# itailang/geometric_adv

Measured on AMD Instinct MI355X. Metric: attack-iterations/sec (B=32, N=2048) at 1/2/4/8 GPUs; Chamfer rel-err vs ref, higher is better.
Workload: dtype f32 (encoder products: f16x2); 1 GPU; BASELINE configs[1]: B=32 random clouds x N=2048, output-space attack (chamfer/chamfer, dist_weight 1.0, lr 0.01), one batch per GPU; batch_per_gpu=32, n_points=2048, global_batch=32, parallelism=batches sharded, dp1, no data-path collective, ranks=1, collective_backend=none, collective_world=1

## Files before the change

geometric_adv_amd/adv_ae.py:

```python
import ctypes as C
import time

import numpy as np
import torch

from . import _lib
from .adversary import init_pert_value
from .autoencoder import PointNetAE


class Configuration:

    def __init__(self, batch_size, n_points, weights, loss="chamfer", loss_adv_type="chamfer",
                 loss_dist_type="chamfer", dist_weight_list=(1.0,), max_point_pert_weight=0.0,
                 max_point_dist_weight=0.0, num_iterations=500, num_iterations_thresh=400,
                 learning_rate=0.01, ae_name="autoencoder", emd_weight=0.0, verbose=False, batch_slots=1,
                 chamfer_prune=True, emd_reference_weights=False, recompute_backward=False, separate_adam=False,
                 chamfer_kernel="auto", encoder_backward="auto", emd_dense_levels=False, encoder_arith=None, loss_in_scan=True):
        self.batch_size = int(batch_size)
        self.n_input = [int(n_points), 3]
        self.n_output = [int(n_points), 3]
        self.weights = weights
        self.loss = loss
        self.loss_adv_type = loss_adv_type
# ... 142 lines not shown
            return None
        if 2 * handed_back > self.B:
            self.set_source_search(False)
        return handed_back

    def status(self):
        with torch.cuda.device(self.device):
            _lib.check(_lib.lib().geoadv_attack_status(self._h, _lib.stream_handle()), "attack_status")

    def peek(self):
        B, n, dev = self.B, self.n, self.device
        f = lambda *s: torch.empty(s, dtype=torch.float32, device=dev)
        i = lambda *s: torch.empty(s, dtype=torch.int32, device=dev)
        out = dict(pert=f(B, n, 3), adv=f(B, n, 3), recon=f(B, n, 3), latent=f(B, 128), grad=f(B, n, 3),
                   idx_r1=i(B, n), idx_r2=i(B, n), idx_a1=i(B, n), idx_a2=i(B, n))
        with torch.cuda.device(dev):
            _lib.check(_lib.lib().geoadv_attack_peek(self._h, *[_lib.ptr(out[k]) for k in
                       ("pert", "adv", "recon", "latent", "grad", "idx_r1", "idx_r2", "idx_a1", "idx_a2")],
                       _lib.stream_handle()), "attack_peek")
        if self.ae.bneck != 128:
            out["latent"] = out["latent"][:, :self.ae.bneck].contiguous()
        return out

    def profile(self, classes, stride=1):
        _lib.check(_lib.lib().geoadv_attack_profile_stride(self._h, int(stride)), "attack_profile_stride")
        if classes is True:
            mask = -1
        elif not classes:
            mask = 0
        else:
            mask = sum(1 << PROF_NAMES.index(c) for c in classes)
        _lib.check(_lib.lib().geoadv_attack_profile(self._h, int(mask)), "attack_profile")

    def markers(self, enable=True):
        _lib.check(_lib.lib().geoadv_attack_markers(self._h, int(bool(enable))), "attack_markers")

    def profile_read(self):
        out = {}
        for k, name in enumerate(PROF_NAMES):
            n_, ms = C.c_int(0), C.c_float(0)
            _lib.check(_lib.lib().geoadv_attack_profile_read(self._h, k, C.byref(n_), C.byref(ms)), "attack_profile_read")
            out[name] = (n_.value, ms.value)
        return out

    def reconstruct(self, X, GT=None, compute_loss=True):
        return self.ae.reconstruct(X, GT, compute_loss)
# ... 100 lines not shown
```

geometric_adv_amd/csrc/attack.hip:

```cpp
#include "ae.h"
#include "chamfer_sym.h"
#include "chamfer_grad.h"
#include "chamfer_grid.h"
#include "encoder_jac.h"
#include "decoder_tail.h"
#define LC_STAMP(K, I) GA_STAMP(K, I)
#include "loss_cgrad.h"
#include <dlfcn.h>
#include <limits.h>
#include <math.h>
#include <stdlib.h>
#include <vector>

#pragma clang fp contract(off)

namespace geoadv {

struct ChamferScan { const float *query; const float *target; float *dist; int *idx; int nq, nt; const int *need; };
int launch_chamfer_scans(const ChamferScan *scans, int nscan, int b, hipStream_t stream);
int launch_encoder_jac(const DeviceAE &A, int b, const JacArgs &a, hipStream_t stream);
int launch_encoder_bwd_dense(const DeviceAE &A, int b, const float *adv, const float *z, const int *zcnt, const float *dz,
                             const int *dense_flag, float *g_enc, hipStream_t stream);
int launch_decoder_fc2_bwd(const DeviceAE &A, int b, const float *g_recon, float *partial, hipStream_t stream);
int launch_decoder_tail_dense(const DeviceAE &A, const TailDenseArgs &a, hipStream_t stream);
// ... 40 lines not shown
    r = block_reduce(r, shf, shi);
    if (t == 0) out[b] = r.s3 * (1.0f / (float)n) + r.s4 * (1.0f / (float)m);
}

__global__ __launch_bounds__(CGA_THREADS) void chamfer_grad_attack_kernel(CGradArgs a) {
    extern __shared__ __attribute__((aligned(16))) unsigned lds[];
    const CGradProblem pr = a.pr[blockIdx.y];
    const int b = blockIdx.x, n = a.n;
    const float wb = pr.w ? pr.w[b] : 1.0f;
    const float gd = wb * (1.0f / (float)n);
    GradSide s;
    s.n_own = n; s.n_oth = n;
    s.own = pr.p + (size_t)b * n * 3; s.oth = pr.q + (size_t)b * n * 3;
    s.match_own = pr.idx1 + (size_t)b * n; s.match_oth = pr.idx2 + (size_t)b * n;
    s.gd_own = nullptr; s.gd_oth = nullptr; s.gd_own_s = gd; s.gd_oth_s = gd;
    s.jstar = (pr.jstar && pr.extra_w > 0.f) ? pr.jstar[b] : -1;
    s.extra = wb * pr.extra_w;
    s.gout = pr.g + (size_t)b * n * 3;
    chamfer_grad_side<true, CGA_THREADS>(s, lds, a.P);
}

__global__ __launch_bounds__(CGA_THREADS) void chamfer_grad_attack_fx_kernel(CGradArgs a, int H) {
    extern __shared__ __attribute__((aligned(16))) unsigned fx_lds[];
    cgrad_fx_body(a, blockIdx.y / H, blockIdx.x, blockIdx.y % H, H, fx_lds);
}

__global__ __launch_bounds__(CGA_THREADS) void loss_cgrad_kernel(LossArgs la, CGradArgs ca, int H) {
    extern __shared__ __attribute__((aligned(16))) unsigned lc_lds[];
    GA_STAMP(0, 0);
    loss_cgrad_block(la, ca, H, blockIdx.x, gridDim.x, blockIdx.y, lc_lds);
    GA_STAMP(0, 7);
}

struct AdamArgs {
    int n, B;
    float *pert, *m, *v;
    float *g_enc;
    const float *g_dist;
    const float *w, *losses;
    const int *jstar;
    int loss_dist_type;
    float mp_pert_w;
    float alpha, one_minus_b1, one_minus_b2, eps;
    float *grad_out;
    const float *x;
    float *adv_out;
};
// ... 59 lines not shown
    }
}

}

using namespace geoadv;

struct geoadv_attack {
    const geoadv_ae *ae;
    geoadv_attack_config cfg;
    int B, n;
    void *arena; size_t arena_bytes;
    float *x, *gt, *tz, *w;
    float *pert, *m, *v;
    float *adv, *recon, *g_recon, *g_dist, *g_enc, *grad_last;
    float *r1, *r2, *a1, *a2; int *ir1, *ir2, *ia1, *ia2;
    ForwardScratch fs;
    float *dz, *dec_partial;
    float *losses; int *jstar;
    float *best_err, *best_metrics, *best_adv, *best_recon;
    float *emd_temp, *emd_cost, *emd_g1;
    float *sym_ws;
    unsigned long long *row64;
    bool row64_filled;
    bool cgrad_done;
    bool counted = false;
    bool chamfer_prune;
    int *need_adv[2];
    float *x_box;
    int grid_calls;
    unsigned *masks;
    float *jac;
    bool jac_valid;
    unsigned *tail_ready;
    unsigned tail_epoch;
    unsigned *loss_done;
    unsigned loss_target;
    bool host_loss_force;
    bool host_loss;
    int cus;
    bool chamfer_sym;
    float beta1_pow, beta2_pow;
    bool fwd_valid;
    bool adv_valid;
    bool fuse_adam;
    bool adam_pending;
// ... 61 lines not shown
    ~ProfScope() {
        if (marked) roctx().pop();
        if (!on) return;
        if (!kernel) {
            e1 = at->ev_used++;
            (void)hipEventRecord(at->ev[e1], st);
        }
        at->marks.push_back({which, e0, e1});
    }
};


int do_forward(geoadv_attack *at, float *hist_slot, int keep, hipStream_t st) {
    const DeviceAE &A = at->ae->d;
    const int B = at->B, n = at->n;
    const ChamferScan sc_recon[2] = {{at->recon, at->gt, at->r1, at->ir1, n, n}, {at->gt, at->recon, at->r2, at->ir2, n, n}};
    const ChamferScan sc_adv[2] = {{at->adv, at->x, at->a1, at->ia1, n, n}, {at->x, at->adv, at->a2, at->ia2, n, n}};
    const bool pruned = at->chamfer_prune && chamfer_grid_supports(n, n);
    const bool adv_chamfer = at->cfg.loss_adv_type == GEOADV_LOSS_ADV_CHAMFER;
    const bool dist_chamfer = at->cfg.loss_dist_type == GEOADV_LOSS_DIST_CHAMFER;
    const bool max_term = dist_chamfer && at->cfg.max_point_dist_weight > 0.f;
    const bool loss_fused = (adv_chamfer || dist_chamfer) && !max_term && n <= CG_FX_MAX_N_PLANE;
    const bool merge_in_loss = loss_fused && adv_chamfer && dist_chamfer;
    const bool use_row64 = merge_in_loss && at->chamfer_sym && at->row64 != nullptr && chamfer_sym_packs_rows((long)B * (pruned ? 1 : 2), n, n);
    SymPartials part{nullptr, nullptr, 1, B, false, use_row64 ? at->row64 : nullptr};
    {
        ProfScope ps(at, GEOADV_PROF_ENCODER_FWD, st, true);
        if (int rc = launch_encoder_fwd(A, B, at->x, at->pert, (at->adv_valid && !at->adam_pending) ? nullptr : at->adv, at->fs.pmax,
                                        at->fs.parg, at->fs.pcnt, at->masks, st, ps.start(), ps.stop(),
                                        at->adam_pending ? &at->pending : nullptr)) return rc;
        at->adam_pending = false;
        at->adv_valid = true;
    }
    const bool rides_scan = pruned && chamfer_grid_rides(n) && at->chamfer_sym;
    const bool rides_latent = pruned && chamfer_grid_rides(n) && !at->chamfer_sym;
    const int call = at->grid_calls;
    int *need_new = at->need_adv[rides_scan ? (call + 1) & 1 : 0];
    const int *need_scan = at->need_adv[rides_scan ? call & 1 : 0];
    if (pruned) at->grid_calls++;
    {
        ProfScope ps(at, GEOADV_PROF_DECODER_FWD, st);
        if (pruned && !rides_scan && !rides_latent) {
            if (int rc = launch_chamfer_grid(at->adv, at->x, at->a1, at->ia1, at->a2, at->ia2, B, n, need_new, call, at->x_box, st)) return rc;
        }
        if (rides_latent) {
            if (int rc = launch_latent_decode_and_grid(A, B, at->fs.pmax, at->fs.parg, at->fs.pcnt, at->fs.z, at->fs.crit, at->fs.zcnt,
                                                       at->fs.dense, at->fs.d1, at->fs.d2, at->adv, at->x, at->a1, at->ia1, at->a2,
                                                       at->ia2, n, need_new, call, at->x_box, st)) return rc;
        } else if (int rc = launch_latent_decode(A, B, at->fs.pmax, at->fs.parg, at->fs.pcnt, at->fs.z, at->fs.crit, at->fs.zcnt,
                                                 at->fs.dense, at->fs.d1, at->fs.d2, st)) return rc;
        if (int rc = launch_decoder_fc2(A, B, at->fs.d2, at->recon, st, use_row64 ? at->row64 : nullptr, use_row64 ? 2 * (size_t)B * n : 0)) return rc;
    }
    const JacArgs jargs{n, at->masks, at->fs.crit, at->fs.z, at->fs.dense, at->jac};
    const bool jac_rides = at->jac && at->chamfer_sym;
    at->jac_valid = jac_rides;
    if (at->jac && !jac_rides && at->cfg.encoder_backward == GEOADV_ENC_BWD_JACOBIAN) {
        ProfScope ps(at, GEOADV_PROF_ENCODER_BWD, st);
        if (int rc = launch_encoder_jac(A, B, jargs, st)) return rc;
        at->jac_valid = true;
    }
    auto fill_loss = [&](const SymPartials &p, LossArgs &la, CGradArgs &ca, int &np) {
        la.n = n; la.loss_adv_type = at->cfg.loss_adv_type; la.loss_dist_type = at->cfg.loss_dist_type;
        la.mp_pert_w = at->cfg.max_point_pert_weight; la.mp_dist_w = at->cfg.max_point_dist_weight;
        la.r1 = at->r1; la.r2 = at->r2; la.a1 = at->a1; la.a2 = at->a2; la.pert = at->pert;
        la.z = at->fs.z; la.tz = at->tz; la.w = at->w; la.losses = at->losses; la.jstar = at->jstar;
        la.emd_cost = at->emd_temp ? at->emd_cost : nullptr; la.emd_weight = at->cfg.emd_weight;
        la.dz_latent = at->dz; la.hist = hist_slot; la.keep = keep; la.best_err = at->best_err;
        la.best_metrics = at->best_metrics; la.adv = at->adv; la.recon = at->recon;
        la.best_adv = at->best_adv; la.best_recon = at->best_recon;
        la.part = p; la.a1_need = pruned ? need_scan : nullptr; la.a1_all = pruned ? 0 : 1; la.r1_out = at->r1; la.a1_out = at->a1;
        np = 0;
        if (adv_chamfer) {
            ca.pr[np] = CGradProblem{at->recon, at->gt, at->ir1, at->ir2, at->g_recon, nullptr, nullptr, 0.f};
            if (p.deferred) {
                ca.pr[np].part_d = p.rowpart_d; ca.pr[np].part_i = p.rowpart_i; ca.pr[np].part_slices = p.slices;
                ca.pr[np].part_need = nullptr; ca.pr[np].idx1_out = at->ir1; ca.pr[np].part_w = p.row64;
            }
            ++np;
        }
        if (dist_chamfer) {
            ca.pr[np] = CGradProblem{at->adv, at->x, at->ia1, at->ia2, at->g_dist, at->w, at->jstar, 0.f};
            if (p.deferred) {
                const size_t off = (size_t)B * p.slices * n;
                ca.pr[np].part_d = p.rowpart_d + off; ca.pr[np].part_i = p.rowpart_i + off; ca.pr[np].part_slices = p.slices;
                ca.pr[np].part_need = pruned ? need_scan : nullptr; ca.pr[np].idx1_out = at->ia1;
                ca.pr[np].part_w = p.row64 ? p.row64 + (size_t)B * n : nullptr;
            }
            ++np;
        }
        ca.n = n; ca.P = 0;
    };
    struct LossCtx { void (*fill)(void *, const SymPartials &, LossArgs &, CGradArgs &, int &); void *self; };
// ... 364 lines not shown

extern "C" int geoadv_attack_get_best(geoadv_attack *at, const float *target_ae_loss_ref, float *metrics, float *adv,
                                      float *recon, void *stream) {
    GA_REQUIRE(at, "attack_get_best: null handle");
    hipStream_t st = as_stream(stream);
    const size_t bn3 = (size_t)at->B * at->n * 3;
    if (metrics) {
        GA_REQUIRE(target_ae_loss_ref, "attack_get_best: target_ae_loss_ref is required for the metrics");
        best_metrics_kernel<<<(at->B + 63) / 64, 64, 0, st>>>(at->B, at->best_metrics, at->best_err, target_ae_loss_ref, metrics,
                                                              reinterpret_cast<const int *>(at->tail_ready + at->B));
        GA_LAUNCH_CHECK();
    }
    if (adv) GA_HIP(hipMemcpyAsync(adv, at->best_adv, 4 * bn3, hipMemcpyDeviceToDevice, st));
    if (recon) GA_HIP(hipMemcpyAsync(recon, at->best_recon, 4 * bn3, hipMemcpyDeviceToDevice, st));
    return GEOADV_OK;
}

extern "C" int geoadv_attack_set_source_search(geoadv_attack *at, int on) {
    GA_REQUIRE(at, "attack_set_source_search: null handle");
    at->chamfer_prune = on != 0;
    return GEOADV_OK;
}

extern "C" int geoadv_attack_status(geoadv_attack *at, void *stream) {
    GA_REQUIRE(at, "attack_status: null handle");
    hipStream_t st = as_stream(stream);
    int failed = 0;
    GA_HIP(hipMemcpyAsync(&failed, at->tail_ready + at->B, sizeof(int), hipMemcpyDeviceToHost, st));
    GA_HIP(hipStreamSynchronize(st));
    if (failed) {
        set_error("attack: an in-launch hand-off (decoder backward tail -> dense encoder backward of a cloud with a tied pool "
                  "maximum) timed out since the last set_inputs / init_pert; iterations after it used a stale latent gradient -- "
                  "the results of this run are invalid");
        return GEOADV_EHIP;
    }
    return ae_range_check(at->ae, st, "attack_status");
}

extern "C" int geoadv_attack_peek(geoadv_attack *at, float *pert, float *adv, float *recon, float *latent, float *grad,
                                  int *idx_r1, int *idx_r2, int *idx_a1, int *idx_a2, void *stream) {
    GA_REQUIRE(at, "attack_peek: null handle");
    hipStream_t st = as_stream(stream);
    const size_t bn3 = 4 * (size_t)at->B * at->n * 3, bn = 4 * (size_t)at->B * at->n;
    if (at->adam_pending || (!at->fwd_valid && (adv || recon || latent || idx_r1 || idx_r2 || idx_a1 || idx_a2)))
        if (int rc = do_forward(at, nullptr, 0, st)) return rc;
    if (pert) GA_HIP(hipMemcpyAsync(pert, at->pert, bn3, hipMemcpyDeviceToDevice, st));
// ... 65 lines not shown
```

geometric_adv_amd/csrc/chamfer_sym.h:

```cpp
#pragma once
#include "common.h"

namespace geoadv {

struct ChamferPair {
    const float *p, *q;
    float *dist1; int *idx1;
    float *dist2; int *idx2;
};

struct SymPartials {
    const float *rowpart_d;
    const int *rowpart_i;
    int slices, clouds;
    bool deferred;
    unsigned long long *row64;
};

#ifdef __HIPCC__
__device__ __forceinline__ bool sym_needed(const int *need, int c) {
    if (!need) return true;
    const int4 lo = reinterpret_cast<const int4 *>(need)[2 * c], hi = reinterpret_cast<const int4 *>(need)[2 * c + 1];
    return (lo.x | lo.y | lo.z | lo.w | hi.x | hi.y | hi.z | hi.w) != 0;
}

__device__ __forceinline__ float sym_merge_pick(const float *d, int slices, size_t stride, int &slice) {
    float bd = d[0];
    int bs = 0;
    for (int s0 = 1; s0 < slices; s0 += 8) {
        float vd[8];
#pragma unroll
        for (int u = 0; u < 8; ++u) vd[u] = d[(size_t)(s0 + u < slices ? s0 + u : 0) * stride];
#pragma unroll
        for (int u = 0; u < 8; ++u)
            if (s0 + u < slices && vd[u] < bd) { bd = vd[u]; bs = s0 + u; }
    }
    slice = bs;
    return bd;
}
// ... 14 lines not shown
#pragma unroll
        for (int u = 0; u < 8; ++u) bd = fminf(bd, vd[u]);
    }
    return bd;
}
#endif

struct CGradProblem {
    const float *p, *q;
    const int *idx1, *idx2;
    float *g;
    const float *w;
    const int *jstar;
    float extra_w;
    const float *part_d; const int *part_i; int part_slices; const int *part_need; int *idx1_out;
    const unsigned long long *part_w;
};
int launch_chamfer_grad(const CGradProblem *pr, int np, int B, int n, hipStream_t st);

int launch_nn_nonfinite_fix(int b, int n, const float *xyz1, int m, const float *xyz2, float *dist1, int *idx1, float *dist2,
                            int *idx2, hipStream_t stream);

size_t chamfer_sym_workspace_floats(int pairs, int b, int n, int m);
bool chamfer_sym_packs_rows(long live_groups, int n, int m);
int launch_chamfer_sym(const ChamferPair *pairs, int np, int b, int n, int m, float *workspace, hipStream_t stream);
struct GridArgs;
struct JacRider;
struct LossRider;
int launch_chamfer_sym_loop(const ChamferPair *pairs, int np, int b, int n, int m, float *workspace, const int *need1,
                            const GridArgs *rider, const JacRider *jac, SymPartials *defer, hipStream_t stream, LossRider *loss = nullptr);
bool chamfer_sym_hosts_loss(long live_groups, int b, int n, int m);

}
```

geometric_adv_amd/csrc/chamfer_sym.hip:

```cpp
#include "common.h"
#include "chamfer_grid.h"
#include "encoder_jac.h"
#include "chamfer_sym.h"
#include "chamfer_mx.h"
#include "loss_cgrad.h"
#include <atomic>
#include <limits.h>
#include <math.h>
#include <stdlib.h>

#pragma clang fp contract(off)

namespace geoadv {

struct ChamferSymArgs {
    ChamferPair pr[2];
    int n, m, clouds, pairs;
    int rw, cw;
    int rtiles;
    int C, S, cslices;
    int pair_base, q_clouds;
    float *rowpart_d;
    int *rowpart_i;
    float *colpart_d;
// ... 359 lines not shown
    s.rtiles = cdiv(n, CS_WROWS * s.rw);
    const int cmin = std::max(CS_CMIN, 2 * CS_ROUND * s.cw);
    s.C = CS_CMAX;
    while (s.C > cmin && (long)s.rtiles * cdiv(m, s.C) * groups < kCUs &&
           (s.C > 128 || (long)s.rtiles * cdiv(m, s.C / 2) * groups <= kCUs)) s.C /= 2;
    s.S = 1;
    while (s.cw == 1 && s.S < CS_MAX_STAGES && (long)s.rtiles * cdiv(m, s.C * s.S * 2) * groups >= 4 * kCUs) s.S *= 2;
    s.cslices = cdiv(m, s.C * s.S);
    return s;
}
static size_t sym_group_floats(const SymShape &s, int n, int m) {
    return 2 * (size_t)s.cslices * s.cw * n + (s.rtiles > 1 ? 2 * (size_t)s.rtiles * m : 0);
}

size_t chamfer_sym_workspace_floats(int pairs, int b, int n, int m) {
    size_t per = 0;
    for (int v = 0; v < 4; ++v) {
        for (long g = 1; g <= (long)pairs * b; g *= 2) per = std::max(per, sym_group_floats(sym_shape(g, n, m, (v & 1) != 0, (v & 2) != 0), n, m));
        per = std::max(per, sym_group_floats(sym_shape((long)pairs * b, n, m, (v & 1) != 0, (v & 2) != 0), n, m));
    }
    return (size_t)pairs * b * per + 64;
}

bool chamfer_sym_packs_rows(long live_groups, int n, int m) {
    const SymShape s = sym_shape(live_groups, n, m, true, mx_enabled());
    return s.rtiles == 1 && s.cslices * s.cw > 8;
}

int launch_chamfer_sym_ex(const ChamferPair *pairs, int np, int b, int n, int m, float *workspace, int pair_base,
                          int q_clouds, const int *need1, hipStream_t stream, const GridArgs *rider = nullptr,
                          const JacRider *jac = nullptr, SymPartials *defer = nullptr, bool loop = false, LossRider *loss = nullptr);
int launch_chamfer_sym(const ChamferPair *pairs, int np, int b, int n, int m, float *workspace, hipStream_t stream) {
    return launch_chamfer_sym_ex(pairs, np, b, n, m, workspace, 0, 0, nullptr, stream);
}
int launch_chamfer_sym_loop(const ChamferPair *pairs, int np, int b, int n, int m, float *workspace, const int *need1,
                            const GridArgs *rider, const JacRider *jac, SymPartials *defer, hipStream_t stream, LossRider *loss) {
    return launch_chamfer_sym_ex(pairs, np, b, n, m, workspace, 0, 0, need1, stream, rider, jac, defer, true, loss);
}
bool chamfer_sym_hosts_loss(long live_groups, int b, int n, int m) {
    const SymShape s = sym_shape(live_groups, n, m, true, mx_enabled());
    return !s.mx && s.rtiles == 1 && b % 8 == 0;
}

int launch_chamfer_sym_ex(const ChamferPair *pairs, int np, int b, int n, int m, float *workspace, int pair_base,
                          int q_clouds, const int *need1, hipStream_t stream, const GridArgs *rider, const JacRider *jac,
                          SymPartials *defer, bool loop, LossRider *loss) {
    if (loss) loss->blocks = 0;
    unsigned long long *row64 = defer ? defer->row64 : nullptr;
    if (defer) { defer->slices = 1; defer->rowpart_d = nullptr; defer->rowpart_i = nullptr; defer->clouds = b; defer->deferred = false; defer->row64 = nullptr; }
    if (b <= 0 || np <= 0) return GEOADV_OK;
    ChamferSymArgs a;
    a.need[0] = nullptr; a.need[1] = need1;
    a.pair_base = pair_base; a.q_clouds = q_clouds;
    for (int i = 0; i < np; ++i) a.pr[i] = pairs[i];
    a.n = n; a.m = m; a.clouds = b; a.pairs = np;
    const int np_live = need1 ? 1 : np;
    const SymShape s = sym_shape((long)b * np_live, n, m, loop, mx_enabled());
    a.rw = s.rw; a.cw = s.cw; a.rtiles = s.rtiles; a.C = s.C; a.S = s.S; a.cslices = s.cslices;
    const int rslices = s.cslices * s.cw;
    const size_t groups = (size_t)np * b;
    a.rowpart_d = workspace;
    a.rowpart_i = reinterpret_cast<int *>(workspace + groups * rslices * n);
    a.colpart_d = workspace + 2 * groups * rslices * n;
    a.colpart_i = reinterpret_cast<int *>(a.colpart_d + groups * s.rtiles * m);
    a.row64 = (defer && row64 && s.rtiles == 1 && rslices > 8) ? row64 : nullptr;
    static DeviceOnce attr;
    if (int rc = attr.run([]() -> int {
            const int need = (int)std::max(std::max(std::max(CS_LDS_BYTES, MX_LDS_BYTES), chamfer_grid_lds_bytes(GR_MAX_N)), JAC_LDS_BYTES);
            GA_HIP(hipFuncSetAttribute(reinterpret_cast<const void *>(chamfer_sym_kernel), hipFuncAttributeMaxDynamicSharedMemorySize, need));
            GA_HIP(hipFuncSetAttribute(reinterpret_cast<const void *>(chamfer_mx_kernel<2>), hipFuncAttributeMaxDynamicSharedMemorySize, need));
            GA_HIP(hipFuncSetAttribute(reinterpret_cast<const void *>(chamfer_mx_kernel<4>), hipFuncAttributeMaxDynamicSharedMemorySize, need));
            GA_HIP(hipFuncSetAttribute(reinterpret_cast<const void *>(chamfer_mx_kernel<8>), hipFuncAttributeMaxDynamicSharedMemorySize, need));
            return GEOADV_OK;
        })) return rc;
    unsigned grid = (unsigned)(s.rtiles * s.cslices * 8 * cdiv(b * np, 8));
    a.rider.blocks = 0; a.rider.first_block = 0; a.rider.clouds = 0; a.rider.done = nullptr;
    a.loss.blocks = 0; a.loss.first_block = 0; a.loss.done = nullptr;
    size_t scan_lds = s.mx ? MX_LDS_BYTES : CS_LDS_BYTES;
    const bool host_loss = loss && !s.mx && s.rtiles == 1 && b % 8 == 0 && q_clouds == 0 &&
                           (loss->force || (rider != nullptr && (long)s.rtiles * s.cslices * b * np_live >= 2 * (long)kCUs));
    if (rider) {
        a.rider.g = *rider;
        a.rider.first_block = 0;
        a.rider.blocks = grid_rider_blocks(b);
        a.rider.clouds = b;
        if (host_loss) a.rider.done = loss->done;
        grid += (unsigned)a.rider.blocks;
        scan_lds = std::max(scan_lds, chamfer_grid_lds_bytes(rider->n));
// ... 129 lines not shown
```

geometric_adv_amd/csrc/loss_cgrad.h:

```cpp
#pragma once
#include "common.h"
#include "chamfer_sym.h"
#include <limits.h>
#include <math.h>

#ifndef LC_STAMP
#define LC_STAMP(K, I)
#endif

namespace geoadv {

struct LossArgs {
    int n;
    int loss_adv_type, loss_dist_type;
    float mp_pert_w, mp_dist_w;
    const float *r1, *r2, *a1, *a2;
    const float *pert;
    const float *z, *tz;
    const float *w;
    const float *emd_cost;
    float emd_weight;
    float *losses;
    int *jstar;
    float *dz_latent;
    float *hist;
    int keep;
    float *best_err;
    float *best_metrics;
    const float *adv, *recon;
    float *best_adv, *best_recon;
    SymPartials part;
    const int *a1_need; int a1_all;
    float *r1_out, *a1_out;
};

struct CloudRed { float s1, s2, s3, s4, sp, ma, mp; int ja, jp; };

__device__ __forceinline__ void argmax_merge(float &v, int &i, float ov, int oi) {
    if (ov > v || (ov == v && oi < i)) { v = ov; i = oi; }
}

__device__ __forceinline__ CloudRed block_reduce(CloudRed r, float (*shf)[8], int (*shi)[2]) {
#pragma unroll
    for (int off = 32; off > 0; off >>= 1) {
        r.s1 += __shfl_xor(r.s1, off); r.s2 += __shfl_xor(r.s2, off); r.s3 += __shfl_xor(r.s3, off);
        r.s4 += __shfl_xor(r.s4, off); r.sp += __shfl_xor(r.sp, off);
        argmax_merge(r.ma, r.ja, __shfl_xor(r.ma, off), __shfl_xor(r.ja, off));
        argmax_merge(r.mp, r.jp, __shfl_xor(r.mp, off), __shfl_xor(r.jp, off));
    }
    const int wave = threadIdx.x >> 6, lane = threadIdx.x & 63;
    if (lane == 0) {
        shf[wave][0] = r.s1; shf[wave][1] = r.s2; shf[wave][2] = r.s3; shf[wave][3] = r.s4; shf[wave][4] = r.sp;
        shf[wave][5] = r.ma; shf[wave][6] = r.mp; shi[wave][0] = r.ja; shi[wave][1] = r.jp;
    }
    __syncthreads();
    CloudRed t;
// ... 34 lines not shown
            if (part3) v3 = __uint_as_float((unsigned)(w3[j] >> 32));
        } else {
            v1 = sym_merge_min(p1 + j, a.part.slices, n);
            if (part3) v3 = sym_merge_min(p3 + j, a.part.slices, n);
        }
        m1[j] = v1; a.r1_out[o + j] = v1;
        if (part3) { m3[j] = v3; a.a1_out[o + j] = v3; }
    }
}

__device__ __forceinline__ void loss_metrics_body(const LossArgs &a, const int b, const int B, const float *m1 = nullptr, const float *m3 = nullptr) {
    __shared__ float shf[4][8];
    __shared__ int shi[4][2];
    __shared__ float sh2[4];
    __shared__ int take;
    const int t = threadIdx.x, n = a.n;
    const size_t o = (size_t)b * n;
    CloudRed r;
    r.s1 = r.s2 = r.s3 = r.s4 = r.sp = 0.f;
    r.ma = r.mp = -1.f;
    r.ja = r.jp = INT_MAX;
    const bool part1 = a.part.deferred;
    const bool part3 = part1 && (a.a1_all || (a.a1_need && sym_needed(a.a1_need, b)));
    constexpr int U = 4;
    for (int j0 = t; j0 < n; j0 += U * 256) {
        float v1[U], v2[U], v3[U], v4[U], vx[U], vy[U], vz[U];
#pragma unroll
        for (int u = 0; u < U; ++u) {
            const int j = j0 + u * 256 < n ? j0 + u * 256 : t;
            v1[u] = part1 ? m1[j] : a.r1[o + j];
            v3[u] = part3 ? m3[j] : a.a1[o + j];
            v2[u] = a.r2[o + j]; v4[u] = a.a2[o + j];
            vx[u] = a.pert[(o + j) * 3]; vy[u] = a.pert[(o + j) * 3 + 1]; vz[u] = a.pert[(o + j) * 3 + 2];
        }
#pragma unroll
        for (int u = 0; u < U; ++u) {
            const int j = j0 + u * 256;
            if (j >= n) continue;
            r.s1 += v1[u]; r.s2 += v2[u];
            const float d = v3[u];
            r.s3 += d; r.s4 += v4[u];
            if (d > r.ma) { r.ma = d; r.ja = j; }
            const float p2 = (vx[u] * vx[u] + vy[u] * vy[u]) + vz[u] * vz[u];
            r.sp += p2;
            if (p2 > r.mp) { r.mp = p2; r.jp = j; }
        }
    }
    r = block_reduce(r, shf, shi);
    float ma = r.ma, mp = r.mp;
    const int ja = r.ja, jp = r.jp;
    const float inv_n = 1.0f / (float)n;
    const float loss_ae = r.s1 * inv_n + r.s2 * inv_n;
    const float input_dist = r.s3 * inv_n + r.s4 * inv_n;
    const float pert_sq = r.sp;
    const float loss_pert = sqrtf(pert_sq), loss_max = sqrtf(mp);
    float loss_adv = loss_ae;
// ... 19 lines not shown
        if (a.hist) {
            a.hist[0 * B + b] = loss_adv; a.hist[1 * B + b] = loss_dist; a.hist[2 * B + b] = loss_pert;
            a.hist[3 * B + b] = fourth;   a.hist[4 * B + b] = input_dist; a.hist[5 * B + b] = loss_ae;
        }
        int tk = 0;
        if (a.keep && loss_ae < a.best_err[b]) {
            tk = 1;
            a.best_err[b] = loss_ae;
            a.best_metrics[b * 4 + 0] = loss_adv; a.best_metrics[b * 4 + 1] = loss_dist;
            a.best_metrics[b * 4 + 2] = input_dist; a.best_metrics[b * 4 + 3] = loss_ae;
        }
        take = tk;
    }
    __syncthreads();
    if (take) {
        const size_t base = o * 3;
        for (int e = t; e < 3 * n; e += 256) {
            a.best_adv[base + e] = a.adv[base + e];
            a.best_recon[base + e] = a.recon[base + e];
        }
    }
}

struct CGradArgs { CGradProblem pr[2]; int n, P; };
constexpr int CGA_THREADS = 512;

constexpr double CG_FX = 17592186044416.0;
constexpr int CG_FX_MAX_N = 5000;
constexpr int CG_FX_MAX_N_PLANE = 15000;
inline int cgrad_fx_parts(int n) { return (n + CG_FX_MAX_N - 1) / CG_FX_MAX_N; }
inline int cgrad_fx_range(int n) { return (n + cgrad_fx_parts(n) - 1) / cgrad_fx_parts(n); }
inline size_t cgrad_fx_lds_bytes(int n) { return sizeof(unsigned long long) * 3 * (size_t)cgrad_fx_range(n); }

__device__ __forceinline__ void cgrad_fx_body(const CGradArgs &a, const int pi, const int b, const int h, const int H, unsigned *lds) {
    unsigned long long *acc = reinterpret_cast<unsigned long long *>(lds);
    const CGradProblem pr = a.pr[pi];
    const int n = a.n;
    const float wb = pr.w ? pr.w[b] : 1.0f;
    const float gd = wb * (1.0f / (float)n);
    const float g2 = gd * 2;
    const float *p = pr.p + (size_t)b * n * 3, *q = pr.q + (size_t)b * n * 3;
    const int *i1 = pr.idx1 + (size_t)b * n, *i2 = pr.idx2 + (size_t)b * n;
    const bool part = (pr.part_d || pr.part_w) && (!pr.part_need || sym_needed(pr.part_need, b));
    const float *pd = pr.part_d + (size_t)b * pr.part_slices * n;
    const int *pi_ = pr.part_i + (size_t)b * pr.part_slices * n;
    const unsigned long long *pw = pr.part_w + (size_t)b * n;
    const int js = (pr.jstar && pr.extra_w > 0.f) ? pr.jstar[b] : -1;
// ... 79 lines not shown
        }
        float qv[U][3], pv[U][3];
#pragma unroll
        for (int u = 0; u < U; ++u) {
            const int j = j0 + u * CGA_THREADS < j_hi ? j0 + u * CGA_THREADS : j_lo;
#pragma unroll
            for (int c = 0; c < 3; ++c) { pv[u][c] = p[3 * j + c]; qv[u][c] = q[3 * mj[u] + c]; }
        }
#pragma unroll
        for (int u = 0; u < U; ++u) {
            const int j = j0 + u * CGA_THREADS;
            if (j >= j_hi) continue;
            const float gown = (j == js ? gd + wb * pr.extra_w : gd) * 2;
#pragma unroll
            for (int c = 0; c < 3; ++c) {
                const float own = gown * (pv[u][c] - qv[u][c]);
                const float sc = (float)((double)(long long)acc[3 * (j - j_lo) + c] * (1.0 / CG_FX));
                pr.g[((size_t)b * n + j) * 3 + c] = own - sc;
            }
        }
    }
}

inline size_t loss_cgrad_lds_bytes(int n) { return std::max(cgrad_fx_lds_bytes(n), sizeof(float) * 2 * (size_t)LOSS_PRE_MAX_N); }
__device__ __forceinline__ void loss_cgrad_block(const LossArgs &la, const CGradArgs &ca, const int H, const int b, const int B, const int row, unsigned *dyn) {
    if (row == 0) {
        float *m1 = reinterpret_cast<float *>(dyn), *m3 = m1 + LOSS_PRE_MAX_N;
        if (la.part.deferred) {
            loss_premerge(la, b, B, CGA_THREADS, m1, m3);
            __syncthreads();
        }
        if (threadIdx.x < 256) loss_metrics_body(la, b, B, m1, m3);
    } else {
        LC_STAMP(1, 0);
        cgrad_fx_body(ca, (row - 1) / H, b, (row - 1) % H, H, dyn);
        LC_STAMP(1, 7);
    }
}

struct LossRider {
    LossArgs la; CGradArgs ca;
    int H, rows, first_block, blocks, clouds;
    unsigned *done;
    unsigned target;
    int *spin_timeout;
    void (*patch)(LossRider &, const SymPartials &, void *);
    void *ctx;
    bool force;
};
inline int loss_rider_blocks(int clouds, int rows) { return 8 * ((clouds + 7) / 8) * rows; }
__device__ __forceinline__ bool loss_rider_block(const LossRider &r, unsigned *dyn) {
    if (r.blocks == 0 || (int)blockIdx.x < r.first_block || (int)blockIdx.x >= r.first_block + r.blocks) return false;
    const int l = blockIdx.x - r.first_block;
    const int idx = l >> 3, row = idx % r.rows, b = (idx / r.rows) * 8 + (l & 7);
    if (b >= r.clouds) return true;
#ifdef GA_STAMPS
#define LR_STAMP(I) do { if (threadIdx.x == 0 && l < GA_STAMP_BLOCKS) { unsigned long long t_; asm volatile("s_memrealtime %0\n\ts_waitcnt lgkmcnt(0)" : "=s"(t_)::"memory"); ga_stamps[((4 & 7) * GA_STAMP_BLOCKS + l) * 8 + (I)] = t_; } } while (0)
#else
// ... 26 lines not shown
```

include/geoadv.h:

```cpp
#ifndef GEOADV_H
#define GEOADV_H

#include <stddef.h>

#ifdef __cplusplus
extern "C" {
#endif

#define GEOADV_OK      0
#define GEOADV_EINVAL  1
#define GEOADV_EHIP    2
#define GEOADV_ENOMEM  3
#define GEOADV_ERANGE  4

int         geoadv_version(void);
const char *geoadv_last_error(void);


int geoadv_nn_distance(int b, int n, const float *xyz1, int m, const float *xyz2,
                       float *dist1, int *idx1, float *dist2, int *idx2, void *stream);

size_t geoadv_nn_distance_sym_workspace_floats(int b, int n, int m);
int geoadv_nn_distance_sym_is_screened(int b, int n, int m);
int geoadv_set_chamfer_screen(int on);
// ... 350 lines not shown
#define GEOADV_CHAMFER_TWO_SCAN  1
#define GEOADV_CHAMFER_SYMMETRIC 2

int  geoadv_attack_create(geoadv_attack **out, const geoadv_ae *ae, const geoadv_attack_config *cfg);
void geoadv_attack_destroy(geoadv_attack *at);

int geoadv_attack_set_inputs(geoadv_attack *at, const float *source_pc, const float *target_pc,
                             const float *target_latent, const float *dist_weight, void *stream);
int geoadv_attack_init_pert(geoadv_attack *at, const float *init_pert, int reset_optimizer, void *stream);

int geoadv_attack_run(geoadv_attack *at, int first_iteration, int iterations, int thresh,
                      float *metrics_hist, void *stream);

int geoadv_attack_get_best(geoadv_attack *at, const float *target_ae_loss_ref,
                           float *metrics, float *adv, float *recon, void *stream);

int geoadv_attack_set_source_search(geoadv_attack *at, int on);

int geoadv_attack_status(geoadv_attack *at, void *stream);

int geoadv_attack_peek(geoadv_attack *at, float *pert, float *adv, float *recon, float *latent,
                       float *grad, int *idx_r1, int *idx_r2, int *idx_a1, int *idx_a2, void *stream);

int geoadv_attack_search_state(geoadv_attack *at, int *searched, int *handed_back, void *stream);

typedef struct geoadv_trainer geoadv_trainer;
typedef struct geoadv_train_config {
    int   batch;
    float learning_rate;
    float bn_decay;
    int   loss;
    int   max_workgroups;
} geoadv_train_config;
#define GEOADV_TRAIN_LOSS_CHAMFER 0
#define GEOADV_TRAIN_LOSS_EMD     1

int  geoadv_trainer_create(geoadv_trainer **out, const geoadv_ae_weights *init, const geoadv_train_config *cfg);
void geoadv_trainer_destroy(geoadv_trainer *t);
int geoadv_trainer_step(geoadv_trainer *t, const float *x, const float *gt, float *loss, float *recon, void *stream);
int geoadv_trainer_forward_backward(geoadv_trainer *t, const float *x, const float *gt, float *loss, float *recon, void *stream);
int geoadv_trainer_apply(geoadv_trainer *t, float grad_scale, void *stream);
int geoadv_trainer_set_world(geoadv_trainer *t, int world);
int geoadv_trainer_num_phases(void);
int geoadv_trainer_run_phase(geoadv_trainer *t, int phase, const float *x, const float *gt, void *stream);
int geoadv_trainer_exchange(geoadv_trainer *t, int phase, double **buf, size_t *count);
int geoadv_trainer_fetch(geoadv_trainer *t, float *loss, float *recon, void *stream);
// ... 34 lines not shown
```

Measured before the change: 8575 attack-iterations/sec.

## Read packed row64 words directly in loss metrics and add single-pass Chamfer gradient

The loss-metrics block now reads merged row minima straight from the packed row64 words instead of premerging the slice partials into LDS, and it writes r1/a1 out as it goes. The row64 packing threshold changes from more than 8 slices to at least 8, so packing covers one more shape. A new single-pass fixed-point Chamfer gradient path holds each thread's points in registers and does one LDS atomic scatter when H==1 and n<=2048. Test hooks can force the old forms; this adds register pressure and a new code path whose numerics must match the old one.

```diff
diff --git a/geometric_adv_amd/adv_ae.py b/geometric_adv_amd/adv_ae.py
--- a/geometric_adv_amd/adv_ae.py
+++ b/geometric_adv_amd/adv_ae.py
@@ -188,6 +188,18 @@
             out["latent"] = out["latent"][:, :self.ae.bneck].contiguous()
         return out
 
+    def _test_loss_form(self, form):
+        _lib.check(_lib.lib().geoadv_attack_test_loss_form(self._h, int(form)), "attack_test_loss_form")
+
+    def _test_loss_state(self):
+        B, n, dev = self.B, self.n, self.device
+        f = lambda *s: torch.empty(s, dtype=torch.float32, device=dev)
+        out = dict(g_recon=f(B, n, 3), g_dist=f(B, n, 3), losses=f(8, B), dist_r1=f(B, n), dist_a1=f(B, n))
+        with torch.cuda.device(dev):
+            _lib.check(_lib.lib().geoadv_attack_test_loss_state(self._h, *[_lib.ptr(out[k]) for k in
+                       ("g_recon", "g_dist", "losses", "dist_r1", "dist_a1")], _lib.stream_handle()), "attack_test_loss_state")
+        return out
+
     def profile(self, classes, stride=1):
         _lib.check(_lib.lib().geoadv_attack_profile_stride(self._h, int(stride)), "attack_profile_stride")
         if classes is True:
diff --git a/geometric_adv_amd/csrc/attack.hip b/geometric_adv_amd/csrc/attack.hip
--- a/geometric_adv_amd/csrc/attack.hip
+++ b/geometric_adv_amd/csrc/attack.hip
@@ -86,7 +86,7 @@
 
 __global__ __launch_bounds__(CGA_THREADS) void chamfer_grad_attack_fx_kernel(CGradArgs a, int H) {
     extern __shared__ __attribute__((aligned(16))) unsigned fx_lds[];
-    cgrad_fx_body(a, blockIdx.y / H, blockIdx.x, blockIdx.y % H, H, fx_lds);
+    cgrad_fx(a, blockIdx.y / H, blockIdx.x, blockIdx.y % H, H, fx_lds);
 }
 
 __global__ __launch_bounds__(CGA_THREADS) void loss_cgrad_kernel(LossArgs la, CGradArgs ca, int H) {
@@ -192,6 +192,7 @@
     float *emd_temp, *emd_cost, *emd_g1;
     float *sym_ws;
     unsigned long long *row64;
+    int test_loss_form = 0;
     bool row64_filled;
     bool cgrad_done;
     bool counted = false;
@@ -299,8 +300,9 @@
     const bool max_term = dist_chamfer && at->cfg.max_point_dist_weight > 0.f;
     const bool loss_fused = (adv_chamfer || dist_chamfer) && !max_term && n <= CG_FX_MAX_N_PLANE;
     const bool merge_in_loss = loss_fused && adv_chamfer && dist_chamfer;
-    const bool use_row64 = merge_in_loss && at->chamfer_sym && at->row64 != nullptr && chamfer_sym_packs_rows((long)B * (pruned ? 1 : 2), n, n);
-    SymPartials part{nullptr, nullptr, 1, B, false, use_row64 ? at->row64 : nullptr};
+    const int pack_from = (at->test_loss_form & 1) ? SYM_PACK_FROM + 1 : SYM_PACK_FROM;
+    const bool use_row64 = merge_in_loss && at->chamfer_sym && at->row64 != nullptr && chamfer_sym_packs_rows((long)B * (pruned ? 1 : 2), n, n, pack_from);
+    SymPartials part{nullptr, nullptr, 1, B, false, use_row64 ? at->row64 : nullptr, pack_from};
     {
         ProfScope ps(at, GEOADV_PROF_ENCODER_FWD, st, true);
         if (int rc = launch_encoder_fwd(A, B, at->x, at->pert, (at->adv_valid && !at->adam_pending) ? nullptr : at->adv, at->fs.pmax,
@@ -345,6 +347,7 @@
         la.dz_latent = at->dz; la.hist = hist_slot; la.keep = keep; la.best_err = at->best_err;
         la.best_metrics = at->best_metrics; la.adv = at->adv; la.recon = at->recon;
         la.best_adv = at->best_adv; la.best_recon = at->best_recon;
+        la.fold_in_lds = (at->test_loss_form & 2) ? 1 : 0; ca.general = la.fold_in_lds;
         la.part = p; la.a1_need = pruned ? need_scan : nullptr; la.a1_all = pruned ? 0 : 1; la.r1_out = at->r1; la.a1_out = at->a1;
         np = 0;
         if (adv_chamfer) {
@@ -755,6 +758,28 @@
     return GEOADV_OK;
 }
 
+extern "C" int geoadv_attack_test_loss_form(geoadv_attack *at, int form) {
+    GA_REQUIRE(at && form >= 0 && form <= 3, "attack_test_loss_form: bad arguments");
+    at->test_loss_form = form;
+    return GEOADV_OK;
+}
+
+extern "C" int geoadv_attack_test_loss_state(geoadv_attack *at, float *g_recon, float *g_dist, float *losses, float *dist_r1,
+                                             float *dist_a1, void *stream) {
+    GA_REQUIRE(at, "attack_test_loss_state: null handle");
+    hipStream_t st = as_stream(stream);
+    const size_t bn3 = 4 * (size_t)at->B * at->n * 3, bn = 4 * (size_t)at->B * at->n;
+    if (at->adam_pending || !at->fwd_valid)
+        if (int rc = do_forward(at, nullptr, 0, st)) return rc;
+    GA_REQUIRE(at->cgrad_done || !(g_recon || g_dist), "attack_test_loss_state: this configuration forms the Chamfer gradients in the step");
+    if (g_recon) GA_HIP(hipMemcpyAsync(g_recon, at->g_recon, bn3, hipMemcpyDeviceToDevice, st));
+    if (g_dist) GA_HIP(hipMemcpyAsync(g_dist, at->g_dist, bn3, hipMemcpyDeviceToDevice, st));
+    if (losses) GA_HIP(hipMemcpyAsync(losses, at->losses, 4 * 8 * (size_t)at->B, hipMemcpyDeviceToDevice, st));
+    if (dist_r1) GA_HIP(hipMemcpyAsync(dist_r1, at->r1, bn, hipMemcpyDeviceToDevice, st));
+    if (dist_a1) GA_HIP(hipMemcpyAsync(dist_a1, at->a1, bn, hipMemcpyDeviceToDevice, st));
+    return GEOADV_OK;
+}
+
 extern "C" int geoadv_attack_status(geoadv_attack *at, void *stream) {
     GA_REQUIRE(at, "attack_status: null handle");
     hipStream_t st = as_stream(stream);
diff --git a/geometric_adv_amd/csrc/chamfer_sym.h b/geometric_adv_amd/csrc/chamfer_sym.h
--- a/geometric_adv_amd/csrc/chamfer_sym.h
+++ b/geometric_adv_amd/csrc/chamfer_sym.h
@@ -9,12 +9,14 @@
     float *dist2; int *idx2;
 };
 
+constexpr int SYM_PACK_FROM = 8;
 struct SymPartials {
     const float *rowpart_d;
     const int *rowpart_i;
     int slices, clouds;
     bool deferred;
     unsigned long long *row64;
+    int pack_from = SYM_PACK_FROM;
 };
 
 #ifdef __HIPCC__
@@ -75,7 +77,7 @@
                             int *idx2, hipStream_t stream);
 
 size_t chamfer_sym_workspace_floats(int pairs, int b, int n, int m);
-bool chamfer_sym_packs_rows(long live_groups, int n, int m);
+bool chamfer_sym_packs_rows(long live_groups, int n, int m, int pack_from = SYM_PACK_FROM);
 int launch_chamfer_sym(const ChamferPair *pairs, int np, int b, int n, int m, float *workspace, hipStream_t stream);
 struct GridArgs;
 struct JacRider;
diff --git a/geometric_adv_amd/csrc/chamfer_sym.hip b/geometric_adv_amd/csrc/chamfer_sym.hip
--- a/geometric_adv_amd/csrc/chamfer_sym.hip
+++ b/geometric_adv_amd/csrc/chamfer_sym.hip
@@ -405,9 +405,9 @@
     return (size_t)pairs * b * per + 64;
 }
 
-bool chamfer_sym_packs_rows(long live_groups, int n, int m) {
+bool chamfer_sym_packs_rows(long live_groups, int n, int m, int pack_from) {
     const SymShape s = sym_shape(live_groups, n, m, true, mx_enabled());
-    return s.rtiles == 1 && s.cslices * s.cw > 8;
+    return s.rtiles == 1 && s.cslices * s.cw >= pack_from;
 }
 
 int launch_chamfer_sym_ex(const ChamferPair *pairs, int np, int b, int n, int m, float *workspace, int pair_base,
@@ -430,6 +430,7 @@
                           SymPartials *defer, bool loop, LossRider *loss) {
     if (loss) loss->blocks = 0;
     unsigned long long *row64 = defer ? defer->row64 : nullptr;
+    const int pack_from = defer ? defer->pack_from : SYM_PACK_FROM;
     if (defer) { defer->slices = 1; defer->rowpart_d = nullptr; defer->rowpart_i = nullptr; defer->clouds = b; defer->deferred = false; defer->row64 = nullptr; }
     if (b <= 0 || np <= 0) return GEOADV_OK;
     ChamferSymArgs a;
@@ -446,7 +447,7 @@
     a.rowpart_i = reinterpret_cast<int *>(workspace + groups * rslices * n);
     a.colpart_d = workspace + 2 * groups * rslices * n;
     a.colpart_i = reinterpret_cast<int *>(a.colpart_d + groups * s.rtiles * m);
-    a.row64 = (defer && row64 && s.rtiles == 1 && rslices > 8) ? row64 : nullptr;
+    a.row64 = (defer && row64 && s.rtiles == 1 && rslices >= pack_from) ? row64 : nullptr;
     static DeviceOnce attr;
     if (int rc = attr.run([]() -> int {
             const int need = (int)std::max(std::max(std::max(CS_LDS_BYTES, MX_LDS_BYTES), chamfer_grid_lds_bytes(GR_MAX_N)), JAC_LDS_BYTES);
diff --git a/geometric_adv_amd/csrc/loss_cgrad.h b/geometric_adv_amd/csrc/loss_cgrad.h
--- a/geometric_adv_amd/csrc/loss_cgrad.h
+++ b/geometric_adv_amd/csrc/loss_cgrad.h
@@ -32,6 +32,7 @@
     SymPartials part;
     const int *a1_need; int a1_all;
     float *r1_out, *a1_out;
+    int fold_in_lds = 0;
 };
 
 struct CloudRed { float s1, s2, s3, s4, sp, ma, mp; int ja, jp; };
@@ -112,16 +113,32 @@
     r.ja = r.jp = INT_MAX;
     const bool part1 = a.part.deferred;
     const bool part3 = part1 && (a.a1_all || (a.a1_need && sym_needed(a.a1_need, b)));
+    const bool words = part1 && m1 == nullptr;
+    const unsigned long long *w1 = a.part.row64 + o, *w3 = a.part.row64 + (size_t)B * n + o;
     constexpr int U = 4;
     for (int j0 = t; j0 < n; j0 += U * 256) {
         float v1[U], v2[U], v3[U], v4[U], vx[U], vy[U], vz[U];
 #pragma unroll
         for (int u = 0; u < U; ++u) {
             const int j = j0 + u * 256 < n ? j0 + u * 256 : t;
-            v1[u] = part1 ? m1[j] : a.r1[o + j];
-            v3[u] = part3 ? m3[j] : a.a1[o + j];
+            if (words) {
+                v1[u] = __uint_as_float((unsigned)(w1[j] >> 32));
+                v3[u] = part3 ? __uint_as_float((unsigned)(w3[j] >> 32)) : a.a1[o + j];
+            } else {
+                v1[u] = part1 ? m1[j] : a.r1[o + j];
+                v3[u] = part3 ? m3[j] : a.a1[o + j];
+            }
             v2[u] = a.r2[o + j]; v4[u] = a.a2[o + j];
             vx[u] = a.pert[(o + j) * 3]; vy[u] = a.pert[(o + j) * 3 + 1]; vz[u] = a.pert[(o + j) * 3 + 2];
+        }
+        if (words) {
+#pragma unroll
+            for (int u = 0; u < U; ++u) {
+                const int j = j0 + u * 256;
+                if (j >= n) continue;
+                a.r1_out[o + j] = v1[u];
+                if (part3) a.a1_out[o + j] = v3[u];
+            }
         }
 #pragma unroll
         for (int u = 0; u < U; ++u) {
@@ -187,7 +204,7 @@
     }
 }
 
-struct CGradArgs { CGradProblem pr[2]; int n, P; };
+struct CGradArgs { CGradProblem pr[2]; int n, P; int general = 0; };
 constexpr int CGA_THREADS = 512;
 
 constexpr double CG_FX = 17592186044416.0;
@@ -313,18 +330,102 @@
     }
 }
 
+constexpr int CG_FX_U = 4;
+__device__ __forceinline__ void cgrad_fx_body_1pass(const CGradArgs &a, const int pi, const int b, unsigned *lds) {
+    unsigned long long *acc = reinterpret_cast<unsigned long long *>(lds);
+    const CGradProblem pr = a.pr[pi];
+    const int n = a.n;
+    const float wb = pr.w ? pr.w[b] : 1.0f;
+    const float gd = wb * (1.0f / (float)n);
+    const float g2 = gd * 2;
+    const float *p = pr.p + (size_t)b * n * 3, *q = pr.q + (size_t)b * n * 3;
+    const int *i1 = pr.idx1 + (size_t)b * n, *i2 = pr.idx2 + (size_t)b * n;
+    const bool part = (pr.part_d || pr.part_w) && (!pr.part_need || sym_needed(pr.part_need, b));
+    const float *pd = pr.part_d + (size_t)b * pr.part_slices * n;
+    const int *pi_ = pr.part_i + (size_t)b * pr.part_slices * n;
+    const unsigned long long *pw = pr.part_w + (size_t)b * n;
+    const int js = (pr.jstar && pr.extra_w > 0.f) ? pr.jstar[b] : -1;
+    constexpr int U = CG_FX_U;
+    int jc[U], jj[U], mj[U];
+    float po[U][3], qo[U][3];
+#pragma unroll
+    for (int u = 0; u < U; ++u) {
+        const int j = threadIdx.x + u * CGA_THREADS;
+        jc[u] = j < n ? j : 0;
+        jj[u] = i2[jc[u]];
+#pragma unroll
+        for (int c = 0; c < 3; ++c) { po[u][c] = p[3 * jc[u] + c]; qo[u][c] = q[3 * jc[u] + c]; }
+    }
+    if (part && pr.part_w) {
+#pragma unroll
+        for (int u = 0; u < U; ++u) mj[u] = (int)(unsigned)pw[jc[u]];
+    } else if (part) {
+        int sl[U];
+#pragma unroll
+        for (int u = 0; u < U; ++u) (void)sym_merge_pick(pd + jc[u], pr.part_slices, n, sl[u]);
+#pragma unroll
+        for (int u = 0; u < U; ++u) mj[u] = pi_[(size_t)sl[u] * n + jc[u]];
+    } else {
+#pragma unroll
+        for (int u = 0; u < U; ++u) mj[u] = i1[jc[u]];
+    }
+    for (int e = threadIdx.x; e < 3 * n; e += CGA_THREADS) acc[e] = 0ull;
+    float qm[U][3], ps[U][3];
+#pragma unroll
+    for (int u = 0; u < U; ++u) {
+#pragma unroll
+        for (int c = 0; c < 3; ++c) { qm[u][c] = q[3 * mj[u] + c]; ps[u][c] = p[3 * jj[u] + c]; }
+    }
+    if (part) {
+#pragma unroll
+        for (int u = 0; u < U; ++u)
+            if (threadIdx.x + u * CGA_THREADS < n) pr.idx1_out[(size_t)b * n + jc[u]] = mj[u];
+    }
+    __syncthreads();
+    LC_STAMP(1, 1);
+#pragma unroll
+    for (int u = 0; u < U; ++u) {
+        if (threadIdx.x + u * CGA_THREADS >= n) continue;
+#pragma unroll
+        for (int c = 0; c < 3; ++c) {
+            const float t = g2 * (qo[u][c] - ps[u][c]);
+            const long long f = __double2ll_rn((double)t * CG_FX);
+            atomicAdd(&acc[3 * jj[u] + c], (unsigned long long)f);
+        }
+    }
+    __syncthreads();
+    LC_STAMP(1, 2);
+#pragma unroll
+    for (int u = 0; u < U; ++u) {
+        const int j = threadIdx.x + u * CGA_THREADS;
+        if (j >= n) continue;
+        const float gown = (j == js ? gd + wb * pr.extra_w : gd) * 2;
+#pragma unroll
+        for (int c = 0; c < 3; ++c) {
+            const float own = gown * (po[u][c] - qm[u][c]);
+            const float sc = (float)((double)(long long)acc[3 * j + c] * (1.0 / CG_FX));
+            pr.g[((size_t)b * n + j) * 3 + c] = own - sc;
+        }
+    }
+}
+__device__ __forceinline__ void cgrad_fx(const CGradArgs &a, const int pi, const int b, const int h, const int H, unsigned *lds) {
+    if (H == 1 && a.n <= CG_FX_U * CGA_THREADS && !a.general) cgrad_fx_body_1pass(a, pi, b, lds);
+    else cgrad_fx_body(a, pi, b, h, H, lds);
+}
+
 inline size_t loss_cgrad_lds_bytes(int n) { return std::max(cgrad_fx_lds_bytes(n), sizeof(float) * 2 * (size_t)LOSS_PRE_MAX_N); }
 __device__ __forceinline__ void loss_cgrad_block(const LossArgs &la, const CGradArgs &ca, const int H, const int b, const int B, const int row, unsigned *dyn) {
     if (row == 0) {
         float *m1 = reinterpret_cast<float *>(dyn), *m3 = m1 + LOSS_PRE_MAX_N;
-        if (la.part.deferred) {
+        const bool fold = la.part.deferred && (la.part.row64 == nullptr || la.fold_in_lds);
+        if (fold) {
             loss_premerge(la, b, B, CGA_THREADS, m1, m3);
             __syncthreads();
         }
-        if (threadIdx.x < 256) loss_metrics_body(la, b, B, m1, m3);
+        if (threadIdx.x < 256) loss_metrics_body(la, b, B, fold ? m1 : nullptr, m3);
     } else {
         LC_STAMP(1, 0);
-        cgrad_fx_body(ca, (row - 1) / H, b, (row - 1) % H, H, dyn);
+        cgrad_fx(ca, (row - 1) / H, b, (row - 1) % H, H, dyn);
         LC_STAMP(1, 7);
     }
 }
diff --git a/include/geoadv.h b/include/geoadv.h
--- a/include/geoadv.h
+++ b/include/geoadv.h
@@ -396,6 +396,10 @@
 int geoadv_attack_peek(geoadv_attack *at, float *pert, float *adv, float *recon, float *latent,
                        float *grad, int *idx_r1, int *idx_r2, int *idx_a1, int *idx_a2, void *stream);
 
+int geoadv_attack_test_loss_form(geoadv_attack *at, int form);
+int geoadv_attack_test_loss_state(geoadv_attack *at, float *g_recon, float *g_dist, float *losses, float *dist_r1, float *dist_a1,
+                                  void *stream);
+
 int geoadv_attack_search_state(geoadv_attack *at, int *searched, int *handed_back, void *stream);
 
 typedef struct geoadv_trainer geoadv_trainer;
```

Result: faster. 8799 attack-iterations/sec (median of 6 runs) (+2.6%).
